# intel/QATzip

Measured on AMD Instinct MI355X. Metric: compress + decompress GB/s (input bytes), QZ_DEFLATE_GZIP_EXT L1, 64 KB chunks, higher is better.
Workload: dtype u8

## Files before the change

### qatzip_amd/csrc/qzk_deflate_lz77.h

```cpp
#ifndef QZK_DEFLATE_LZ77_H
#define QZK_DEFLATE_LZ77_H
#include "qzk_common.h"
#include "qzk_crcmath.h"

#define QZK_WSIZE 32768
#define QZK_MAXDIST 32506
#define QZK_MINLOOK 262
#define QZK_LITBUF 32767
#define QZK_MAXBLK 20
#define QZK_CAP 16
#define QZK_WLIM 61
#define QZK_NICE 8
#define QZK_MAXINS 4
#define QZK_HSIZE 65536
#ifndef QZK_CNBLOG
#define QZK_CNBLOG (-1)
#endif
#if QZK_CNBLOG >= 0
#define QZK_CNB (1 << QZK_CNBLOG)
#else
#define QZK_CNB 0
#endif
#ifndef QZK_PF
#define QZK_PF (QZK_CNB ? 1 : 0)
#endif
#ifndef QZK_PF_MINL
#define QZK_PF_MINL 30
#endif
#ifndef QZK_NSLOT
#define QZK_NSLOT 256
#endif
#ifndef QZK_RING
#define QZK_RING 4096
#endif
#ifndef QZK_K1_OCC
#define QZK_K1_OCC 5
#endif
#define QZK_RINGW (QZK_RING / 4)
#ifndef QZK_NSLOT2
#define QZK_NSLOT2 128
#endif
#ifndef QZK_NSLOT3
#if QZK_CNB
#define QZK_NSLOT3 0
#else
#define QZK_NSLOT3 128
#endif
#endif
#define QZK_K1_PARSEW (2 * QZK_NSLOT + QZK_RINGW + 4 + QZK_NSLOT2 + QZK_NSLOT3 + 3 * QZK_CNB)
#ifndef QZK_K1_WAVES
#define QZK_K1_WAVES 4
#endif

#ifndef QZK_K1_TABGRP
#define QZK_K1_TABGRP 5
#endif
#define QZK_K1_TABW (QZK_K1_WAVES * QZK_K1_TABGRP)
#define QZK_K1_TABROWS(wgs) ((((wgs) + 8u * QZK_K1_TABGRP - 1) / (8u * QZK_K1_TABGRP)) * 8u)

typedef struct __attribute__((aligned(16))) { uint32_t w0, w1, w2, ep; } qzk_bkt;
typedef uint32_t qzk_u32x4 __attribute__((vector_size(16)));

QZ_DEV qzk_u32x4 qzk_ld_bkt(const qzk_bkt *p)
{
#ifdef QZ_SIM
    return *(const qzk_u32x4 *)p;
#else
    qzk_u32x4 v;
    asm volatile("global_load_dwordx4 %0, %1, off sc1\n\ts_waitcnt vmcnt(0)" : "=v"(v) : "v"(p) : "memory");
    return v;
#endif
}

QZ_DEV void qzk_ld_bkt_ahead(qzk_u32x4 *v, const qzk_bkt *p)
{
#ifdef QZ_SIM
    *v = *(const qzk_u32x4 *)p;
#else
    asm volatile("global_load_dwordx4 %0, %1, off sc1" : "+v"(*v) : "v"(p) : "memory");
#endif
}
QZ_DEV void qzk_wait_ahead(qzk_u32x4 *v)
{
#ifdef QZ_SIM
    (void)v;
#else
    asm volatile("s_waitcnt vmcnt(0)" : "+v"(*v) : : "memory");
#endif
}

#ifdef QZ_SIM
static unsigned long qzk_sim_count[2];
#define QZK_SIMC(k) do { if (qz_lane() == 0) qzk_sim_count[k]++; } while (0)
#else
#define QZK_SIMC(k) do { } while (0)
#endif
#if defined(QZK_PROF) && !defined(QZ_SIM)
#define QZK_T(k) do { uint64_t t_ = __builtin_readcyclecounter(); prof[k] += t_ - tprev; tprev = t_; } while (0)
#define QZK_C(k, v) do { prof[k] += (uint64_t)(v); } while (0)
#else
#define QZK_T(k) do { } while (0)
#define QZK_C(k, v) do { } while (0)
#endif

typedef struct {
    uint32_t nsym;
    uint32_t nfull;
    uint32_t bstart[QZK_MAXBLK];
    uint32_t can_store;
    uint32_t n;
#ifdef QZK_PROF
    uint64_t prof[24];
#endif
} qzk_lzmeta;

#define QZK_CDESC_FINAL 0x80000000u
QZ_DEV uint32_t qzk_chunk_len(const uint32_t *cdesc, uint32_t chunk, uint64_t src_len, uint32_t chunk_sz)
{
    if (cdesc) return cdesc[chunk] & ~QZK_CDESC_FINAL;
    const uint64_t coff = (uint64_t)chunk * chunk_sz;
    return (uint32_t)((src_len - coff) < chunk_sz ? (src_len - coff) : chunk_sz);
}

QZ_DEV uint32_t qzk_ld32g(const uint8_t *src, uint64_t off, uint64_t src_len)
{
    if (off + 4 <= src_len) return qz_ld32(src + off);
    uint32_t v = 0;
    for (int k = 0; k < 4; k++) if (off + k < src_len) v |= (uint32_t)src[off + k] << (8 * k);
    return v;
}

QZ_DEV uint32_t qzk_ld32g_fast(const uint8_t *src, uint64_t off, uint64_t src_len)
{
    return off + 4 <= src_len ? qz_ld32(src + off) : qzk_ld32g(src, off, src_len);
}

QZ_DEV uint32_t qzk_alignbyte(uint32_t hi, uint32_t lo, uint32_t s)
{
#ifdef QZ_SIM
    return (uint32_t)((((uint64_t)hi << 32) | lo) >> (8 * s));
#else
    return __builtin_amdgcn_alignbyte(hi, lo, s);
#endif
}

QZ_DEV int qzk_wave_matchlen(const uint8_t *src, uint64_t src_len, uint64_t a, uint64_t b, int maxlen, int lane)
{
    for (int off = 0; off < maxlen; off += 256) {
        int o = off + 4 * lane;
        bool act = o < maxlen;
        uint32_t x = 0;
        if (act) x = qzk_ld32g(src, a + o, src_len) ^ qzk_ld32g(src, b + o, src_len);
        uint64_t mm = qz_ballot(act && x != 0);
        if (mm) {
            int f = qz_ctz64(mm);
            uint32_t xf = qz_readlane(x, f);
            int len = off + 4 * f + (qz_ctz32(xf) >> 3);
            return len < maxlen ? len : maxlen;
        }
    }
    return maxlen;
}

QZ_DEV void qzk_lz77_chunk(const uint8_t *src, uint64_t src_len, uint32_t chunk_sz, uint32_t chunk,
                           uint8_t *sym_lc, uint16_t *sym_dist, qzk_lzmeta *meta, qzk_bkt *tab, uint32_t epoch,
                           const uint32_t *cdesc, uint32_t *lds, const qzk_k1crc_lds *crcT, uint32_t *crc_slot)
{
    uint32_t *const slot = lds, *const scnt = lds + QZK_NSLOT, *const ring = lds + 2 * QZK_NSLOT, *const slot2 = ring + QZK_RINGW + 4;
    uint32_t *const slot3 = slot2 + QZK_NSLOT2; (void)slot3;
#if QZK_CNB
    uint32_t *const ctag = slot3 + QZK_NSLOT3, *const cpos = ctag + QZK_CNB;
#pragma nounroll
    for (uint32_t i = (uint32_t)qz_lane(); i < QZK_CNB; i += 64) ctag[i] = 0;
#endif
    uint32_t rhi = 0;
    uint32_t crc_acc = 0;
    uint32_t rnext = qzk_ld32g_fast(src, (uint64_t)chunk * chunk_sz + 4 * (uint32_t)qz_lane(), src_len);
#define QZK_RING16(dst, ca) do { const uint32_t r_ = (ca) & (QZK_RING - 1), i_ = r_ >> 2, s_ = r_ & 3; \
        const uint32_t d0_ = ring[i_], d1_ = ring[i_ + 1], d2_ = ring[i_ + 2], d3_ = ring[i_ + 3], d4_ = ring[i_ + 4]; \
        (dst)[0] = qzk_alignbyte(d1_, d0_, s_); (dst)[1] = qzk_alignbyte(d2_, d1_, s_); \
        (dst)[2] = qzk_alignbyte(d3_, d2_, s_); (dst)[3] = qzk_alignbyte(d4_, d3_, s_); } while (0)
#define QZK_RING4(ca) ({ const uint32_t r_ = (ca) & (QZK_RING - 1), i_ = r_ >> 2; \
        qzk_alignbyte(ring[i_ + 1], ring[i_], r_ & 3); })
#define QZK_AHEAD (64 + 258 + 6)

    const int lane = qz_lane();
    const uint64_t coff = (uint64_t)chunk * chunk_sz;
    const uint32_t n = qzk_chunk_len(cdesc, chunk, src_len, chunk_sz);
    uint8_t *olc = sym_lc;
    uint16_t *odist = sym_dist;
    qzk_lzmeta *mt = meta + chunk;
    auto wave_matchlen = [&](uint32_t ca, uint32_t cb, int maxlen) -> int {
        const bool near = (int64_t)cb >= (int64_t)rhi - QZK_RING;
        for (int off = 0; off < maxlen; off += 256) {
            const int o = off + 4 * lane;
            const bool act = o < maxlen;
            uint32_t x = 0;
            if (act) x = QZK_RING4(ca + (uint32_t)o) ^ (near ? QZK_RING4(cb + (uint32_t)o) : qzk_ld32g(src, coff + cb + (uint32_t)o, src_len));
            const uint64_t mm = qz_ballot(act && x != 0);
            if (mm) {
                const int f = qz_ctz64(mm);
                const uint32_t xf = qz_readlane(x, f);
                const int len = off + 4 * f + (qz_ctz32(xf) >> 3);
                return len < maxlen ? len : maxlen;
            }
        }
        return maxlen;
    };

    qz_lds_sync();

    uint32_t base = 0;
    uint32_t fill = n < 65536u ? n : 65536u;
    uint32_t avail_in = n - fill;
    uint32_t pos = 0;
    uint32_t nsym = 0, nfull = 0, cur_bstart = 0, can_store = 0;
    mt->bstart[0] = 0;
#if QZK_PF
    qzk_u32x4 pf = {0, 0, 0, 0};
    uint64_t pf_okm = 0;
    uint32_t pf_base = 0, pf_mark = 0, wcount = 0;
    bool pf_lost = false;
    uint64_t dPm = 0, dSTm = 0;
    uint32_t dnsym = 0, dv_sym = 0, dv_h = 0, dv_e0 = 0, dv_e1 = 0, dv_e2 = 0;
#define QZK_DEFERRED_STORES() do { \
        if ((dPm >> lane) & 1) { const uint32_t i_ = dnsym + (uint32_t)qz_popc64(dPm & qz_below(lane)); \
                                 olc[i_] = (uint8_t)dv_sym; odist[i_] = (uint16_t)(dv_sym >> 8); } \
        if ((dSTm >> lane) & 1) { const qzk_u32x4 e_ = {dv_e0, dv_e1, dv_e2, epoch}; *(qzk_u32x4 *)&tab[(size_t)dv_h * QZK_K1_TABW] = e_; } \
        dPm = 0; dSTm = 0; } while (0)
    bool pf_live = false;
#endif
#if defined(QZK_PROF) && !defined(QZ_SIM)
    uint64_t prof[24] = {0}; uint64_t tprev = __builtin_readcyclecounter();
#endif

    for (;;) {
        uint32_t look = fill - pos;
        if (look < QZK_MINLOOK) {
            if (pos - base >= (uint32_t)(QZK_WSIZE + QZK_MAXDIST)) {
                base += QZK_WSIZE;
#if QZK_CNB
                qz_lds_sync();
#pragma nounroll
                for (uint32_t i = (uint32_t)lane; i < 2 * QZK_CNB; i += 64) {
                    const uint32_t v = cpos[i];
                    const int a = (int)(v & 0xffffu) - QZK_WSIZE, b = (int)(v >> 16) - QZK_WSIZE;
                    cpos[i] = (uint32_t)(a > 0 ? a : 0) | (uint32_t)(b > 0 ? b : 0) << 16;
                }
                qz_lds_sync();
#endif
            }
            if (avail_in) {
                uint32_t more = 65536u - (fill - base);
                uint32_t rd = avail_in < more ? avail_in : more;
                fill += rd; avail_in -= rd;
            }
            look = fill - pos;
            if (look == 0) break;
        }

        QZK_T(0); QZK_C(8, 1);
#if QZK_PF
        qzk_wait_ahead(&pf);
        QZK_T(17);
        QZK_DEFERRED_STORES();
        QZK_T(18);
#endif
        const uint32_t B = pos - base;
        const uint32_t p = B + (uint32_t)lane;
        const uint32_t pa = pos + (uint32_t)lane;
        const int avail = pa < fill ? (int)(fill - pa) : 0;
        const bool canh = avail >= 3;
        const bool guard = coff + pos + 64 + 2 * QZK_CAP > src_len;
        uint32_t w0 = 0, w1 = 0, w2 = 0, w3 = 0;
        {
            if (rhi < pos + QZK_AHEAD) {
                do {
                    const uint32_t a = rhi + 4 * (uint32_t)lane;
                    const uint32_t ri = (a >> 2) & (QZK_RINGW - 1);
                    ring[ri] = rnext;
                    if (ri < 4) ring[ri + QZK_RINGW] = rnext;
                    if (crcT && a + 4 <= n) crc_acc = qzk_k1crc_step(crcT, crc_acc, rnext);
                    rhi += 256;
                    rnext = qzk_ld32g_fast(src, coff + a + 256, src_len);
                } while (rhi < pos + QZK_AHEAD);
                qz_lds_sync();
            }
            uint32_t w[4];
            QZK_RING16(w, pa);
            w0 = w[0]; w1 = w[1]; w2 = w[2]; w3 = w[3];
        }
        const uint32_t h = (((w0 & 0xf) << 12) ^ (((w0 >> 8) & 0xff) << 6) ^ ((w0 >> 16) & 0xff)) & 0xffff;
        const uint32_t bucket = h;
        const uint32_t key = h & (QZK_NSLOT - 1);

        int nvalid = look < 64 ? (int)look : 64;
        int lim = nvalid < QZK_WLIM ? nvalid : QZK_WLIM;
        {
            int lstop;
            int first_short = (int)look - (QZK_MINLOOK - 1);
            if (first_short < 0) first_short = 0;
            if (avail_in) lstop = first_short;
            else {
                int sl = (int)(QZK_WSIZE + QZK_MAXDIST) - (int)B;
                lstop = first_short > sl ? first_short : sl;
            }
            if (lstop < 1) lstop = 1;
            if (lim > lstop) lim = lstop;
        }
        QZK_T(1);
        qz_lds_sync();
        qzk_u32x4 ev = {0, 0, 0, 0};
#if QZK_CNB
        const uint32_t cset = ((h * 40503u) >> (16 - QZK_CNBLOG)) & (QZK_CNB - 1);
        const uint32_t ct = ctag[cset], cp0 = cpos[cset], cp1 = cpos[QZK_CNB + cset];
        const bool chit = canh && ct == (h | 0x10000u);
        QZK_C(8, (uint64_t)qz_popc64(qz_ballot(chit)) << 32);
#if QZK_PF
        bool evhave = false;
        int limdata = 64;
        {
            const uint32_t sh = pos - pf_base;
            if (pf_live && !pf_lost && sh < 64u - (QZK_PF_MINL + 3)) {
                const int sl = lane + (int)sh;
                const uint32_t a0 = qz_shfl(pf[0], sl), a1 = qz_shfl(pf[1], sl), a2 = qz_shfl(pf[2], sl), a3 = qz_shfl(pf[3], sl);
                if (canh && !chit && sl < 64 && ((pf_okm >> (sl & 63)) & 1) && slot[key] != (pf_mark | h) && scnt[(h >> 8) & (QZK_NSLOT - 1)] != (pf_mark | h)) {
                    ev[0] = a0; ev[1] = a1; ev[2] = a2; ev[3] = a3; evhave = true;
                }
            }
            const bool lack = canh && !chit && !evhave;
            const uint64_t LACK = qz_ballot(lack);
            if (LACK) {
                const int fl = qz_ctz64(LACK);
                if (fl < QZK_PF_MINL + 3) { if (lack) { ev = qzk_ld_bkt(&tab[(size_t)bucket * QZK_K1_TABW]); evhave = true; } QZK_C(15, 1ull << 32); QZK_SIMC(0); }
                else limdata = fl - 3;
            }
        }
#else
        const bool evhave = canh && !chit;
        if (canh && !chit) ev = qzk_ld_bkt(&tab[(size_t)bucket * QZK_K1_TABW]);
#endif
#if QZK_PF
        if (lim > limdata) lim = limdata;
        QZK_SIMC(1);
#endif
        QZK_T(16);
        const bool ev_ok = ev[3] == epoch;
        uint32_t q0 = ev_ok ? ev[0] & 0xffffffu : 0, q1 = ev_ok ? (ev[0] >> 24) | ((ev[1] & 0xffffu) << 8) : 0,
                 q2 = ev_ok ? (ev[1] >> 16) | ((ev[2] & 0xffu) << 16) : 0, q3 = ev_ok ? ev[2] >> 8 : 0;
        if (chit) {
            q0 = (cp0 & 0xffffu) ? base + (cp0 & 0xffffu) : 0; q1 = (cp0 >> 16) ? base + (cp0 >> 16) : 0;
            q2 = (cp1 & 0xffffu) ? base + (cp1 & 0xffffu) : 0; q3 = (cp1 >> 16) ? base + (cp1 >> 16) : 0;
        }
#else
        if (canh) ev = qzk_ld_bkt(&tab[(size_t)bucket * QZK_K1_TABW]);
        const bool ev_ok = ev[3] == epoch;
        const uint32_t q0 = ev_ok ? ev[0] & 0xffffffu : 0, q1 = ev_ok ? (ev[0] >> 24) | ((ev[1] & 0xffffu) << 8) : 0,
                       q2 = ev_ok ? (ev[1] >> 16) | ((ev[2] & 0xffu) << 16) : 0, q3 = ev_ok ? ev[2] >> 8 : 0;
#endif
        const uint32_t lo = base + (p > QZK_MAXDIST ? p - QZK_MAXDIST : 0);
        const int maxlen = avail < 258 ? avail : 258;
        const int nice = avail < QZK_NICE ? avail : QZK_NICE;
        int best_len = 2; uint32_t best_c = 0;
        int l0 = 0, l1 = 0, l2 = 0, l3 = 0;
        bool suspect;
        int nc; uint32_t c0, c1, c2, c3;
        {
            uint32_t x[4][4];
            const bool ok0 = canh && q0 > base && pa - q0 <= QZK_MAXDIST;
            const bool ok1 = ok0 && q1 > lo;
            const bool ok2 = ok1 && q2 > lo;
            const bool ok3 = ok2 && q3 > lo;
            c0 = ok0 ? q0 : pa; c1 = ok1 ? q1 : pa; c2 = ok2 ? q2 : pa; c3 = ok3 ? q3 : pa;
            QZK_RING16(x[0], c0); QZK_RING16(x[1], c1); QZK_RING16(x[2], c2); QZK_RING16(x[3], c3);
#define QZK_LDF(k, ck) do { const uint32_t ca_ = (ck); if ((int64_t)ca_ < (int64_t)rhi - QZK_RING) { const uint64_t g_ = coff + ca_; \
        if (!guard) { x[k][0] = qz_ld32(src + g_); x[k][1] = qz_ld32(src + g_ + 4); x[k][2] = qz_ld32(src + g_ + 8); x[k][3] = qz_ld32(src + g_ + 12); } \
        else { x[k][0] = qzk_ld32g(src, g_, src_len); x[k][1] = qzk_ld32g(src, g_ + 4, src_len); x[k][2] = qzk_ld32g(src, g_ + 8, src_len); x[k][3] = qzk_ld32g(src, g_ + 12, src_len); } } } while (0)
#ifndef QZK_EXP_NOFAR
            QZK_LDF(0, c0); QZK_LDF(1, c1); QZK_LDF(2, c2); QZK_LDF(3, c3);
#endif
#undef QZK_LDF
            nc = (int)ok0 + (int)ok1 + (int)ok2 + (int)ok3;
            QZK_T(2);
            const uint32_t key2 = (h >> (16 - 8)) & (QZK_NSLOT2 - 1);
#if QZK_NSLOT3
            const uint32_t key3 = ((h * 40503u) >> 12) & (QZK_NSLOT3 - 1);
            if (canh) slot3[key3] = 0xffffffffu;
#endif
            if (canh) { slot[key] = 0xffffffffu; scnt[key] = 0; slot2[key2] = 0xffffffffu; }
            qz_lds_sync();
            if (canh) { atomicMin(&slot[key], ((uint32_t)lane << 16) | h); atomicAdd(&scnt[key], 1u); atomicMin(&slot2[key2], (uint32_t)lane); }
#if QZK_NSLOT3
            if (canh) atomicMin(&slot3[key3], (uint32_t)lane);
#endif
            qz_lds_sync();
            {
                const uint32_t sv = canh ? slot[key] : 0, sc = canh ? scnt[key] : 0, s2 = canh ? slot2[key2] : 0;
                suspect = canh && (sv >> 16) != (uint32_t)lane && !(sc == 2 && (sv & 0xffff) != h) && s2 != (uint32_t)lane;
#if QZK_NSLOT3
                if (suspect && slot3[key3] == (uint32_t)lane) suspect = false;
#endif
            }
            bool done = false;
            for (int k = 0; k < 4; k++) {
                const uint32_t ck = k == 0 ? c0 : k == 1 ? c1 : k == 2 ? c2 : c3;
                int len = 0;
                if (k < nc) {
                    uint32_t d;
                    len = QZK_CAP;
                    d = w3 ^ x[k][3]; if (d) len = 12 + (qz_ctz32(d) >> 3);
                    d = w2 ^ x[k][2]; if (d) len = 8 + (qz_ctz32(d) >> 3);
                    d = w1 ^ x[k][1]; if (d) len = 4 + (qz_ctz32(d) >> 3);
                    d = w0 ^ x[k][0]; if (d) len = (qz_ctz32(d) >> 3);
                    if (len > maxlen) len = maxlen;
                    if (!done) {
                        if (len > best_len) { best_len = len; best_c = ck; }
                        if (len >= nice) done = true;
                    }
                }
                if (k == 0) l0 = len; else if (k == 1) l1 = len; else if (k == 2) l2 = len; else l3 = len;
            }
        }
        uint32_t mlen = best_len >= 3 ? (uint32_t)best_len : 0;
        uint32_t mdist = mlen ? pa - best_c : 0;
        const bool capped = (best_len == QZK_CAP) && (maxlen > QZK_CAP);
        const bool exact0 = nc > 0 && pa - c0 == QZK_MAXDIST;

        QZK_T(3);
        const uint64_t CANH = qz_ballot(canh);
        const uint64_t CAPM = qz_ballot(capped);
        const uint64_t CX = qz_ballot(suspect) | CAPM;
        const uint64_t NOLIT = qz_ballot(mlen != 0) | CX;

        QZK_T(4);
#if QZK_PF
        {
            pf_base = pos + (uint32_t)lim; pf_live = true;
            pf_mark = 0x80000000u | wcount << 16; wcount = (wcount + 1) & 0x7fffu;
            const uint32_t ppa = pf_base + (uint32_t)lane;
            const bool pcanh = ppa + 3 <= fill;
            const uint32_t pw = QZK_RING4(ppa);
            const uint32_t ph = (((pw & 0xf) << 12) ^ (((pw >> 8) & 0xff) << 6) ^ ((pw >> 16) & 0xff)) & 0xffff;
            const uint32_t ps = ((ph * 40503u) >> (16 - QZK_CNBLOG)) & (QZK_CNB - 1);
            const uint32_t pct = ctag[ps], pc0 = cpos[ps], pc1 = cpos[QZK_CNB + ps];
            const uint32_t g0 = (pc0 & 0xffffu) ? base + (pc0 & 0xffffu) : 0, g1 = (pc0 >> 16) ? base + (pc0 >> 16) : 0,
                           g2 = (pc1 & 0xffffu) ? base + (pc1 & 0xffffu) : 0, g3 = (pc1 >> 16) ? base + (pc1 >> 16) : 0;
            pf[0] = g0 | (g1 << 24); pf[1] = (g1 >> 8) | (g2 << 16); pf[2] = (g2 >> 16) | (g3 << 8); pf[3] = epoch;
            if (pcanh && pct != (ph | 0x10000u)) qzk_ld_bkt_ahead(&pf, &tab[(size_t)ph * QZK_K1_TABW]);
            pf_okm = qz_ballot(pcanh);
        }
#endif
        uint64_t Pm = 0;
        uint64_t SHm = qz_ballot(mlen >= 3 && mlen <= QZK_MAXINS && avail - (int)mlen >= 3), S4m = qz_ballot(mlen == 4);
        int l = 0;
        while (l < lim) {
            uint64_t cxr = CX >> l;
            int nextc = cxr ? l + qz_ctz64(cxr) : 64;
            int stop = nextc < lim ? nextc : lim;
            while (l < stop) {
                const uint64_t nl = (NOLIT | (1ull << 63)) >> l;
                int e = l + qz_ctz64(nl);
                if (e > stop) e = stop;
                const uint32_t ml = qz_readlane(mlen, e);
                const int isM = e < stop ? 1 : 0;
                Pm |= ((1ull << (e - l + isM)) - 1) << l;
                l = e + (isM ? (int)ml : 0);
            }
            if (l >= lim || l != nextc) continue;
            QZK_T(5); QZK_C(9, 1);
            {
                const uint32_t h_l = qz_readlane(h, l);
                const uint64_t earlier = qz_ballot(canh && h == h_l) & qz_below(l);
                const uint32_t ml_l = qz_readlane(mlen, l);
                if (earlier == 0 && !((CAPM >> l) & 1)) {
                    QZK_C(15, 1);
                    Pm |= 1ull << l;
                    l += ml_l ? (int)ml_l : 1;
                    QZK_T(6);
                    continue;
                }
                const int avail_l = (int)look - l;
                const int maxlen_l = avail_l < 258 ? avail_l : 258;
                const int nice_l = avail_l < QZK_NICE ? avail_l : QZK_NICE;
                int cnt = 0, bl = 2; uint32_t bd = 0; bool fin = false;
                bool had_intra = false;
                if (earlier) {
                    const uint64_t ps = Pm & SHm;
                    const uint64_t I = (Pm & CANH) | (ps << 1) | (ps << 2) | ((ps & S4m) << 3);
                    uint64_t Sh = earlier & I;
                    if (B == 0) Sh &= ~1ull;
                    had_intra = Sh != 0;
                    if (Sh) {
                        const uint32_t a0 = qz_readlane(w0, l), a1 = qz_readlane(w1, l), a2 = qz_readlane(w2, l), a3 = qz_readlane(w3, l);
                        while (Sh && cnt < 4 && !fin) {
                            int j = qz_msb64(Sh);
                            Sh &= ~(1ull << j);
                            int len = QZK_CAP;
                            {
                                uint32_t d;
                                d = a3 ^ qz_readlane(w3, j); if (d) len = 12 + (qz_ctz32(d) >> 3);
                                d = a2 ^ qz_readlane(w2, j); if (d) len = 8 + (qz_ctz32(d) >> 3);
                                d = a1 ^ qz_readlane(w1, j); if (d) len = 4 + (qz_ctz32(d) >> 3);
                                d = a0 ^ qz_readlane(w0, j); if (d) len = (qz_ctz32(d) >> 3);
                            }
                            if (len > maxlen_l) len = maxlen_l;
                            if (len == QZK_CAP && maxlen_l > QZK_CAP)
                                len = wave_matchlen(pos + (uint32_t)l, pos + (uint32_t)j, maxlen_l);
                            cnt++;
                            if (len > bl) { bl = len; bd = (uint32_t)(l - j); }
                            if (len >= nice_l) fin = true;
                        }
                    }
                }
                const int nc_l = (int)qz_readlane((uint32_t)nc, l);
                const bool ex_l = qz_readlane((uint32_t)exact0, l) != 0;
                if (!fin && !(had_intra && ex_l)) {
                    for (int k = 0; k < nc_l && cnt < 4 && !fin; k++) {
                        const uint32_t ck = qz_readlane(k == 0 ? c0 : k == 1 ? c1 : k == 2 ? c2 : c3, l);
                        int len = (int)qz_readlane((uint32_t)(k == 0 ? l0 : k == 1 ? l1 : k == 2 ? l2 : l3), l);
                        if (len == QZK_CAP && maxlen_l > QZK_CAP)
                            len = wave_matchlen(pos + (uint32_t)l, ck, maxlen_l);
                        cnt++;
                        if (len > bl) { bl = len; bd = (pos + (uint32_t)l) - ck; }
                        if (len >= nice_l) fin = true;
                    }
                }
                uint32_t nl = bl >= 3 ? (uint32_t)bl : 0;
                if (lane == l) { mlen = nl; mdist = nl ? bd : 0; }
                {
                    const uint64_t bit = 1ull << l;
                    SHm = (nl >= 3 && nl <= QZK_MAXINS && avail_l - (int)nl >= 3) ? SHm | bit : SHm & ~bit;
                    S4m = nl == 4 ? S4m | bit : S4m & ~bit;
                }
                Pm |= 1ull << l;
                l += nl ? (int)nl : 1;
            }
            QZK_T(6);
        }

        QZK_T(5);
        const uint64_t ps = Pm & SHm;
        const uint64_t I = (Pm & CANH) | (ps << 1) | (ps << 2) | ((ps & S4m) << 3);
        const bool isP = (Pm >> lane) & 1, isI = (I >> lane) & 1;

        const uint32_t rank = (uint32_t)qz_popc64(Pm & qz_below(lane));
        const uint32_t idx = nsym + rank;
        const uint32_t step = mlen ? mlen : 1;
        if (isP) {
#if QZK_PF
            dv_sym = (mlen ? mlen - 3 : (w0 & 0xff)) | mdist << 8;
#else
            olc[idx] = (uint8_t)(mlen ? mlen - 3 : (w0 & 0xff));
            odist[idx] = (uint16_t)mdist;
#endif
        }
        {
            const bool closes = isP && ((idx + 1) % QZK_LITBUF == 0);
            const uint64_t cm = qz_ballot(closes);
            if (cm) {
                int f = qz_ctz64(cm);
                uint32_t nb = qz_readlane(pa + step, f);
                if (cur_bstart >= base) can_store |= 1u << nfull;
                nfull++;
                cur_bstart = nb;
                if (nfull < QZK_MAXBLK) mt->bstart[nfull] = nb;
            }
        }
#if QZK_PF
        dPm = Pm; dnsym = nsym;
#endif
        nsym += (uint32_t)qz_popc64(Pm);

        QZK_T(7);
        uint32_t n0 = pa, n1 = q0, n2 = q1, n3 = q2;
        bool store = isI;
        {
            uint64_t todo = I & qz_ballot(suspect);
            QZK_C(10, qz_popc64(todo)); QZK_C(11, qz_popc64(Pm));
            while (todo) {
                const int j = qz_msb64(todo);
                uint32_t b_j = qz_readlane(bucket, j);
                const uint64_t same = qz_ballot(canh && bucket == b_j) & I;
                todo &= ~same;
                uint64_t mates = same & qz_below(j);
                uint32_t m1 = 0, m2 = 0, m3 = 0;
                int nf = 1;
                while (mates && nf < 4) {
                    const int m = qz_msb64(mates);
                    mates &= ~(1ull << m);
                    const uint32_t mp = pos + (uint32_t)m;
                    if (nf == 1) m1 = mp; else if (nf == 2) m2 = mp; else m3 = mp;
                    nf++;
                }
                if (lane == j) {
                    if (nf == 2) { n1 = m1; n2 = q0; n3 = q1; }
                    else if (nf == 3) { n1 = m1; n2 = m2; n3 = q0; }
                    else if (nf == 4) { n1 = m1; n2 = m2; n3 = m3; }
                }
                if (((same >> lane) & 1) && lane < j) store = false;
            }
        }
#if QZK_PF
        dSTm = qz_ballot(store); dv_h = bucket;
        dv_e0 = n0 | (n1 << 24); dv_e1 = (n1 >> 8) | (n2 << 16); dv_e2 = (n2 >> 16) | (n3 << 8);
#else
        if (store) {
            const qzk_u32x4 e = {n0 | (n1 << 24), (n1 >> 8) | (n2 << 16), (n2 >> 16) | (n3 << 8), epoch};
            *(qzk_u32x4 *)&tab[(size_t)bucket * QZK_K1_TABW] = e;
        }
#endif
#if QZK_CNB
        {
            const bool ralloc = evhave && !isI;
            const uint32_t mark = (store ? 0x20040u : 0x20000u) | (uint32_t)lane;
#if QZK_PF
            {
                const uint32_t mk = pf_mark | h, key3 = (h >> 8) & (QZK_NSLOT - 1);
                if (store) slot[key] = mk;
                qz_lds_sync();
                const bool second = store && slot[key] != mk;
                if (second) scnt[key3] = mk;
                qz_lds_sync();
                pf_lost = qz_ballot(second && scnt[key3] != mk) != 0;
            }
#endif
            if (ralloc) ctag[cset] = mark;
            qz_lds_sync();
            if (store) ctag[cset] = mark;
            qz_lds_sync();
            if ((store || ralloc) && ctag[cset] == mark) {
                const uint32_t e0 = store ? n0 : q0, e1 = store ? n1 : q1, e2 = store ? n2 : q2, e3 = store ? n3 : q3;
                const uint32_t r0 = e0 > base ? e0 - base : 0, r1 = e1 > base ? e1 - base : 0, r2 = e2 > base ? e2 - base : 0,
                               r3 = e3 > base ? e3 - base : 0;
                cpos[cset] = r0 | r1 << 16; cpos[QZK_CNB + cset] = r2 | r3 << 16;
                ctag[cset] = h | 0x10000u;
            }
        }
#endif
        pos += (uint32_t)l;
        QZK_T(12);
    }

#if QZK_PF
    qzk_wait_ahead(&pf);
    QZK_DEFERRED_STORES();
#undef QZK_DEFERRED_STORES
#endif
    if (crcT) {
        for (; rhi < n; rhi += 256) {
            const uint32_t a = rhi + 4 * (uint32_t)lane;
            if (a + 4 <= n) crc_acc = qzk_k1crc_step(crcT, crc_acc, rnext);
            rnext = qzk_ld32g_fast(src, coff + a + 256, src_len);
        }
        const uint32_t n4 = n & ~3u;
        const uint32_t mine = n4 > 4u * (uint32_t)lane ? (n4 - 4u * (uint32_t)lane + 252u) >> 8 : 0;
        uint32_t part = 0;
        if (mine) part = qzk_multmodp(qzk_x2nmodp(crcT->x2n, n4 - (4u * (uint32_t)lane + 4u + 256u * (mine - 1)), 3), crc_acc);
        for (int d = 32; d >= 1; d >>= 1) part ^= qz_shfl(part, lane ^ d);
        if (n & 3u) {
            uint32_t c = 0xffffffffu;
            for (uint32_t i = n4; i < n; i++) c = qzk_crc_byte(c, src[coff + i]);
            part = qzk_multmodp(qzk_x2nmodp(crcT->x2n, n & 3u, 3), part) ^ ~c;
        }
        *crc_slot = part;
    }
    if (cur_bstart >= base) can_store |= 1u << nfull;
    mt->nsym = nsym; mt->nfull = nfull; mt->can_store = can_store; mt->n = n;
#if defined(QZK_PROF) && !defined(QZ_SIM)
    for (int k = 0; k < 24; k++) mt->prof[k] = prof[k];
#endif
#undef QZK_RING16
#undef QZK_RING4
}

#endif
```

Before: 66.71.

## Precompute single-intra-match candidates in parallel to skip serial per-lane resolution

Adds a default-on SIMPLE path: each lane finds the nearest earlier lane with the same hash via extra LDS atomic rounds, computes that intra-wave match length in parallel with shuffles, and combines it with the hash-chain lengths into a precomputed alternate match. The serial parse loop then takes this precomputed result, or skips the lane when no intra candidate is actually reachable, instead of doing readlane-heavy scalar matching. It also packs the candidate lengths, count and exact flag into one word so a single readlane replaces several. The cost is three extra LDS syncs and shuffle work every step, and match selection may differ slightly from the full path.

```diff
diff --git a/qatzip_amd/csrc/qzk_deflate_lz77.h b/qatzip_amd/csrc/qzk_deflate_lz77.h
--- a/qatzip_amd/csrc/qzk_deflate_lz77.h
+++ b/qatzip_amd/csrc/qzk_deflate_lz77.h
@@ -47,6 +47,9 @@
 #define QZK_NSLOT3 128
 #endif
 #endif
+#ifndef QZK_SIMPLE
+#define QZK_SIMPLE ((QZK_CNB || QZK_PF) ? 0 : 1)
+#endif
 #define QZK_K1_PARSEW (2 * QZK_NSLOT + QZK_RINGW + 4 + QZK_NSLOT2 + QZK_NSLOT3 + 3 * QZK_CNB)
 #ifndef QZK_K1_WAVES
 #define QZK_K1_WAVES 4
@@ -90,7 +93,7 @@
 }
 
 #ifdef QZ_SIM
-static unsigned long qzk_sim_count[2];
+static unsigned long qzk_sim_count[8];
 #define QZK_SIMC(k) do { if (qz_lane() == 0) qzk_sim_count[k]++; } while (0)
 #else
 #define QZK_SIMC(k) do { } while (0)
@@ -259,7 +262,7 @@
             if (look == 0) break;
         }
 
-        QZK_T(0); QZK_C(8, 1);
+        QZK_T(0); QZK_C(8, 1); QZK_SIMC(2);
 #if QZK_PF
         qzk_wait_ahead(&pf);
         QZK_T(17);
@@ -364,6 +367,9 @@
         int best_len = 2; uint32_t best_c = 0;
         int l0 = 0, l1 = 0, l2 = 0, l3 = 0;
         bool suspect;
+#if QZK_SIMPLE
+        uint32_t jrec = 0;
+#endif
         int nc; uint32_t c0, c1, c2, c3;
         {
             uint32_t x[4][4];
@@ -399,6 +405,25 @@
                 suspect = canh && (sv >> 16) != (uint32_t)lane && !(sc == 2 && (sv & 0xffff) != h) && s2 != (uint32_t)lane;
 #if QZK_NSLOT3
                 if (suspect && slot3[key3] == (uint32_t)lane) suspect = false;
+#endif
+#if QZK_SIMPLE
+                const bool later = canh && (sv & 0xffff) == h && (sv >> 16) != (uint32_t)lane;
+                qz_lds_sync();
+                if (later) scnt[key] = 0xffffffffu;
+                qz_lds_sync();
+                if (later) atomicMin(&scnt[key], (uint32_t)lane);
+                qz_lds_sync();
+                const bool second = later && scnt[key] == (uint32_t)lane;
+                if (qz_ballot(second)) {
+                    const int js = second ? (int)(sv >> 16) : lane;
+                    const uint32_t y0 = qz_shfl(w0, js), y1 = qz_shfl(w1, js), y2 = qz_shfl(w2, js), y3 = qz_shfl(w3, js);
+                    uint32_t lenJ = QZK_CAP, d;
+                    d = w3 ^ y3; if (d) lenJ = 12 + (qz_ctz32(d) >> 3);
+                    d = w2 ^ y2; if (d) lenJ = 8 + (qz_ctz32(d) >> 3);
+                    d = w1 ^ y1; if (d) lenJ = 4 + (qz_ctz32(d) >> 3);
+                    d = w0 ^ y0; if (d) lenJ = (qz_ctz32(d) >> 3);
+                    if (second) jrec = 0x8000u | lenJ << 8 | (uint32_t)(lane - js);
+                }
 #endif
             }
             bool done = false;
@@ -425,6 +450,24 @@
         uint32_t mdist = mlen ? pa - best_c : 0;
         const bool capped = (best_len == QZK_CAP) && (maxlen > QZK_CAP);
         const bool exact0 = nc > 0 && pa - c0 == QZK_MAXDIST;
+        const uint32_t lpk = (uint32_t)l0 | (uint32_t)l1 << 5 | (uint32_t)l2 << 10 | (uint32_t)l3 << 15 | (uint32_t)nc << 20 | (uint32_t)exact0 << 23;
+#if QZK_SIMPLE
+        uint32_t alt = 0;
+        uint64_t SIMPLEM = 0;
+        if (qz_ballot(jrec != 0)) {
+            int lenJ = (int)((jrec >> 8) & 0x7fu);
+            if (lenJ > maxlen) lenJ = maxlen;
+            const bool simple = jrec != 0 && !capped && !(lenJ == QZK_CAP && maxlen > QZK_CAP);
+            int bl = 2; uint32_t bd = 0;
+            if (lenJ > bl) { bl = lenJ; bd = jrec & 0xffu; }
+            bool fin = lenJ >= nice || exact0;
+            if (!fin && nc > 0) { if (l0 > bl) { bl = l0; bd = pa - c0; } fin = l0 >= nice; }
+            if (!fin && nc > 1) { if (l1 > bl) { bl = l1; bd = pa - c1; } fin = l1 >= nice; }
+            if (!fin && nc > 2) { if (l2 > bl) { bl = l2; bd = pa - c2; } }
+            if (bl >= 3) alt = (uint32_t)bl | bd << 16;
+            SIMPLEM = qz_ballot(simple);
+        }
+#endif
 
         QZK_T(3);
         const uint64_t CANH = qz_ballot(canh);
@@ -467,19 +510,48 @@
                 l = e + (isM ? (int)ml : 0);
             }
             if (l >= lim || l != nextc) continue;
-            QZK_T(5); QZK_C(9, 1);
+            QZK_T(5); QZK_C(9, 1); QZK_SIMC(3);
             {
                 const uint32_t h_l = qz_readlane(h, l);
                 const uint64_t earlier = qz_ballot(canh && h == h_l) & qz_below(l);
                 const uint32_t ml_l = qz_readlane(mlen, l);
                 if (earlier == 0 && !((CAPM >> l) & 1)) {
-                    QZK_C(15, 1);
+                    QZK_C(15, 1); QZK_SIMC(4);
                     Pm |= 1ull << l;
                     l += ml_l ? (int)ml_l : 1;
                     QZK_T(6);
                     continue;
                 }
                 const int avail_l = (int)look - l;
+#if QZK_SIMPLE
+                {
+                    const uint64_t ps = Pm & SHm;
+                    const uint64_t I = (Pm & CANH) | (ps << 1) | (ps << 2) | ((ps & S4m) << 3);
+                    uint64_t Sh = earlier & I;
+                    if (B == 0) Sh &= ~1ull;
+                    if (Sh == 0 && !((CAPM >> l) & 1)) {
+                        QZK_C(20, 1); QZK_SIMC(6);
+                        Pm |= 1ull << l;
+                        l += ml_l ? (int)ml_l : 1;
+                        QZK_T(6);
+                        continue;
+                    }
+                    if ((SIMPLEM >> l) & 1) {
+                        QZK_C(19, 1); QZK_SIMC(5);
+                        const uint32_t a = qz_readlane(alt, l);
+                        const uint32_t nl = a & 0xffffu;
+                        if (lane == l) { mlen = nl; mdist = a >> 16; }
+                        const uint64_t bit = 1ull << l;
+                        SHm = (nl >= 3 && nl <= QZK_MAXINS && avail_l - (int)nl >= 3) ? SHm | bit : SHm & ~bit;
+                        S4m = nl == 4 ? S4m | bit : S4m & ~bit;
+                        Pm |= bit;
+                        l += nl ? (int)nl : 1;
+                        QZK_T(6);
+                        continue;
+                    }
+                }
+#endif
+                QZK_SIMC(7);
                 const int maxlen_l = avail_l < 258 ? avail_l : 258;
                 const int nice_l = avail_l < QZK_NICE ? avail_l : QZK_NICE;
                 int cnt = 0, bl = 2; uint32_t bd = 0; bool fin = false;
@@ -512,12 +584,13 @@
                         }
                     }
                 }
-                const int nc_l = (int)qz_readlane((uint32_t)nc, l);
-                const bool ex_l = qz_readlane((uint32_t)exact0, l) != 0;
+                const uint32_t lp = qz_readlane(lpk, l);
+                const int nc_l = (int)((lp >> 20) & 7u);
+                const bool ex_l = (lp >> 23) != 0;
                 if (!fin && !(had_intra && ex_l)) {
                     for (int k = 0; k < nc_l && cnt < 4 && !fin; k++) {
                         const uint32_t ck = qz_readlane(k == 0 ? c0 : k == 1 ? c1 : k == 2 ? c2 : c3, l);
-                        int len = (int)qz_readlane((uint32_t)(k == 0 ? l0 : k == 1 ? l1 : k == 2 ? l2 : l3), l);
+                        int len = (int)((lp >> (5 * k)) & 31u);
                         if (len == QZK_CAP && maxlen_l > QZK_CAP)
                             len = wave_matchlen(pos + (uint32_t)l, ck, maxlen_l);
                         cnt++;
```

New measurement: 66.69 (median of 2 runs). No clear change (-0.0%).
